# winstonww/ReacherDistilation

Hardware: AMD Instinct MI355X
Metric: Reacher env-steps/sec (rollout+distill step) at 1/2/4/8 MI355X; student MSE (higher is better)
Workload: dtype f32; 1 GPU; c4; description=BASELINE config 4: 262,144 envs per GPU, RCCL student-grad all-reduce, MSE, fp32, envs_per_gpu=262144, envs_total=262144, student=MlpPolicy 2x64 tanh (5060 params, f32), teacher=MlpPolicy 2x64 tanh, loss=mse, act_with=teacher, optimizer=TF1 Adam lr 0.0001, 1 step per env-step, parallelism=dp1, collective=none, f32_mode=split

## Files before the change

### reacherdistilation_amd/csrc/distill_forward.h

```cpp
#pragma once

#ifdef RD_MFMA_SRCC_FENCE
constexpr bool kFenceAll = true;
#else
constexpr bool kFenceAll = false;
#endif
#include "distill_forward_f32.h"

constexpr unsigned kPairFence = 0x8a00u;
template <bool FENCE = false, unsigned FM = FENCE ? 0xffffu : 0u>
__device__ __forceinline__ void mlp_forward_pair(const float* LT, const float* LS, const float* ob, int j, int g,
                                                 f32x4 (&H1)[4], f32x4 (&H2)[4], float& mt0, float& mt1,
                                                 float& ms0, float& ms1) {
    f32x4 at[4], as[4];
#pragma unroll
    for (int fb = 0; fb < 4; ++fb) at[fb] = as[fb] = f32x4{0.f, 0.f, 0.f, 0.f};
#pragma unroll
    for (int s = 0; s < 3; ++s) {
        const int k = 4 * s + g;
        const float x = ob[j * SOS + k];
        const float zt = fminf(fmaxf((x - LT[N_MU + k]) * LT[N_RS + k], -5.0f), 5.0f);
        const float zs = fminf(fmaxf((x - LS[N_MU + k]) * LS[N_RS + k], -5.0f), 5.0f);
        const f32x4 wt = ld4(LT + N_W1 + k * HID + 4 * j);
        const f32x4 ws = ld4(LS + N_W1 + k * HID + 4 * j);
// ... 87 lines not shown
}
__device__ __forceinline__ bf16x8 ldbf8(const float* base, int half) {
    return *reinterpret_cast<const bf16x8*>(reinterpret_cast<const unsigned short*>(base) + half);
}

__device__ __forceinline__ int kperm(int s, int g, int jj) { return 32 * s + 4 * g + (jj & 3) + 16 * (jj >> 2); }

__device__ void load_net_bf16(float* L, const float* g, int nthreads) {
    unsigned short* w1 = reinterpret_cast<unsigned short*>(L + NB_W1);
    unsigned short* w2f = reinterpret_cast<unsigned short*>(L + NB_W2F);
    unsigned short* w2b = reinterpret_cast<unsigned short*>(L + NB_W2B);
    for (int x = threadIdx.x; x < 4 * 4 * 16 * 8; x += nthreads) {
        const int jj = x & 7, i = (x >> 3) & 15, fb = (x >> 7) & 3, gg = x >> 9;
        const int k = 8 * gg + jj;
        w1[x] = bf16_bits(k < OBD ? g[P_W1 + k * HID + 16 * fb + i] : 0.0f);
    }
    for (int x = threadIdx.x; x < 2 * 4 * 4 * 16 * 8; x += nthreads) {
        const int jj = x & 7, i = (x >> 3) & 15, b = (x >> 7) & 3, gg = (x >> 9) & 3, s = x >> 11;
        const int kp = kperm(s, gg, jj);
        w2f[x] = bf16_bits(g[P_W2 + kp * HID + 16 * b + i]);
        w2b[x] = bf16_bits(g[P_W2 + (16 * b + i) * HID + kp]);
    }
    for (int x = threadIdx.x; x < HID; x += nthreads) {
        L[NB_B1 + x] = g[P_B1 + x];
        L[NB_B2 + x] = g[P_B2 + x];
    }
    for (int x = threadIdx.x; x < HID * ACD; x += nthreads) L[NB_W3 + x] = bf16_round(g[P_W3 + x]);
    if (threadIdx.x < ACD) {
        L[NB_B3 + threadIdx.x] = g[P_B3 + threadIdx.x];
        L[NB_LS + threadIdx.x] = g[P_LS + threadIdx.x];
    }
    if (threadIdx.x < 12) {
        const int k = threadIdx.x;
        L[NB_MU + k] = k < OBD ? g[P_TOT + k] : 0.0f;
        L[NB_RS + k] = k < OBD ? 1.0f / g[P_TOT + OBD + k] : 1.0f;
    }
}

typedef unsigned u32x4 __attribute__((ext_vector_type(4)));

__device__ __forceinline__ void split1(float x, unsigned short (&h)[3]) {
    const uint32_t u = __float_as_uint(x);
    const float r = x - __uint_as_float(u & 0xffff0000u);
    const uint32_t ur = __float_as_uint(r);
    const float l = r - __uint_as_float(ur & 0xffff0000u);
    h[0] = (unsigned short)(u >> 16);
    h[1] = (unsigned short)(ur >> 16);
    h[2] = (unsigned short)(__float_as_uint(l) >> 16);
}

__device__ __forceinline__ void split_bits(float x, uint32_t& u0, uint32_t& u1, uint32_t& u2) {
    u0 = __float_as_uint(x);
    const float r = x - __uint_as_float(u0 & 0xffff0000u);
    u1 = __float_as_uint(r);
    u2 = __float_as_uint(r - __uint_as_float(u1 & 0xffff0000u));
}

__device__ __forceinline__ void split8(f32x4 lo, f32x4 hi, bf16x8 (&p)[3]) {
    const float x[8] = {lo[0], lo[1], lo[2], lo[3], hi[0], hi[1], hi[2], hi[3]};
    uint32_t u0[8], u1[8], u2[8];
#pragma unroll
    for (int i = 0; i < 8; ++i) split_bits(x[i], u0[i], u1[i], u2[i]);
    u32x4 q0, q1, q2;
#pragma unroll
    for (int i = 0; i < 4; ++i) {
        q0[i] = __builtin_amdgcn_perm(u0[2 * i + 1], u0[2 * i], 0x07060302u);
        q1[i] = __builtin_amdgcn_perm(u1[2 * i + 1], u1[2 * i], 0x07060302u);
        q2[i] = __builtin_amdgcn_perm(u2[2 * i + 1], u2[2 * i], 0x07060302u);
    }
    p[0] = __builtin_bit_cast(bf16x8, q0);
    p[1] = __builtin_bit_cast(bf16x8, q1);
    p[2] = __builtin_bit_cast(bf16x8, q2);
}

__device__ __forceinline__ uint32_t pair_hi(uint32_t a, uint32_t b) { return __builtin_amdgcn_perm(b, a, 0x07060302u); }

__device__ __forceinline__ f32x4 mfma_split(const bf16x8 (&w)[3], const bf16x8 (&x)[3], f32x4 c) {
    c = mfma_k32(w[2], x[0], c);
    c = mfma_k32(w[1], x[1], c);
    c = mfma_k32(w[0], x[2], c);
    c = mfma_k32(w[1], x[0], c);
    c = mfma_k32(w[0], x[1], c);
    return mfma_k32(w[0], x[0], c);
}

typedef float f32x16 __attribute__((ext_vector_type(16)));
__device__ __forceinline__ f32x16 mfma_32k16(bf16x8 a, bf16x8 b, f32x16 c) {
    return __builtin_amdgcn_mfma_f32_32x32x16_bf16(a, b, c, 0, 0, 0);
}
__device__ __forceinline__ void dw2_split32(const float (&x)[2][8], const float (&y)[2][8], f32x16 (&g)[2][2]) {
    bf16x8 xp[2][3], yp[2][3];
#pragma unroll
    for (int b = 0; b < 2; ++b) {
        split8(f32x4{x[b][0], x[b][1], x[b][2], x[b][3]}, f32x4{x[b][4], x[b][5], x[b][6], x[b][7]}, xp[b]);
        split8(f32x4{y[b][0], y[b][1], y[b][2], y[b][3]}, f32x4{y[b][4], y[b][5], y[b][6], y[b][7]}, yp[b]);
    }
#pragma unroll
    for (int mb = 0; mb < 2; ++mb)
#pragma unroll
        for (int nb = 0; nb < 2; ++nb) {
            f32x16 c = g[mb][nb];
            c = mfma_32k16(xp[mb][2], yp[nb][0], c);
            c = mfma_32k16(xp[mb][1], yp[nb][1], c);
            c = mfma_32k16(xp[mb][0], yp[nb][2], c);
            c = mfma_32k16(xp[mb][1], yp[nb][0], c);
            c = mfma_32k16(xp[mb][0], yp[nb][1], c);
            g[mb][nb] = mfma_32k16(xp[mb][0], yp[nb][0], c);
        }
}

__device__ __forceinline__ void ld_pieces(const float* L, int base, int o, bf16x8 (&w)[3]) {
    const unsigned short* h = reinterpret_cast<const unsigned short*>(L + base);
#pragma unroll
    for (int q = 0; q < 3; ++q) w[q] = *reinterpret_cast<const bf16x8*>(h + q * SP_PIECE + o);
}

__device__ __forceinline__ void layer1_split(const float* L, const float* ob, int j, int g, f32x4 (&acc)[4]) {
    u32x4 b[3];
#pragma unroll
    for (int s = 0; s < 3; ++s) {
        const int k = 4 * s + g;
        const float z = fminf(fmaxf((ob[j * SOS + k] - L[NX_MU + k]) * L[NX_RS + k], -5.0f), 5.0f);
        uint32_t z0, z1, z2;
        split_bits(z, z0, z1, z2);
        b[0][s] = pair_hi(z2, z0);
        b[1][s] = pair_hi(z1, z1);
        b[2][s] = pair_hi(z0, z0);
    }
#pragma unroll
    for (int q = 0; q < 3; ++q) {
        b[q][3] = 0u;
        const bf16x8 bq = __builtin_bit_cast(bf16x8, b[q]);
#pragma unroll
        for (int fb = 0; fb < 4; ++fb)
            acc[fb] = mfma_k32(ldbf8(L + NX_W1S, ((((q ? 1 : 0) * 4 + g) * 4 + fb) * 16 + j) * 8), bq, acc[fb]);
    }
}

__device__ __forceinline__ void mlp_forward_pair_split(const float* LT, const float* LS, const float* ob, int j, int g,
                                                       f32x4 (&H1)[4], f32x4 (&H2)[4], float& mt0, float& mt1,
                                                       float& ms0, float& ms1) {
    f32x4 at[4], as[4];
#pragma unroll
    for (int fb = 0; fb < 4; ++fb) at[fb] = as[fb] = f32x4{0.f, 0.f, 0.f, 0.f};
    layer1_split(LT, ob, j, g, at);
    layer1_split(LS, ob, j, g, as);
    f32x4 T1[4];
#pragma unroll
    for (int fb = 0; fb < 4; ++fb) {
        T1[fb] = tanh4(at[fb]);
        H1[fb] = tanh4(as[fb]);
    }
#pragma unroll
    for (int fb = 0; fb < 4; ++fb) {
        at[fb] = ld4(LT + NX_B2 + 16 * fb + 4 * g);
        as[fb] = ld4(LS + NX_B2 + 16 * fb + 4 * g);
    }
    {
        bf16x8 tp[2][3], sp[2][3];
        __builtin_amdgcn_sched_barrier(0);
        split8(T1[0], T1[1], tp[0]);
        split8(H1[0], H1[1], sp[0]);
        __builtin_amdgcn_sched_barrier(0);
        split8(T1[2], T1[3], tp[1]);
        split8(H1[2], H1[3], sp[1]);
#pragma unroll
// ... 276 lines not shown
```

### reacherdistilation_amd/csrc/distill_layout.h

```cpp
#pragma once

constexpr int OBD = 11, HID = 64, ACD = 2;
constexpr int P_W1 = 0;
constexpr int P_B1 = P_W1 + OBD * HID;
constexpr int P_W2 = P_B1 + HID;
constexpr int P_B2 = P_W2 + HID * HID;
constexpr int P_W3 = P_B2 + HID;
constexpr int P_B3 = P_W3 + HID * ACD;
constexpr int P_LS = P_B3 + ACD;
constexpr int P_TOT = P_LS + ACD;
constexpr int P_PAD = P_TOT + 4;
constexpr int N_MET = 4;

constexpr int WAVES = 8, BLOCK = 64 * WAVES;
constexpr int FWAVES = 4, FBLOCK = 64 * FWAVES;
constexpr int GROUP = 64;
constexpr int TILE = 16;

constexpr int N_W1 = 0;
constexpr int N_W2 = N_W1 + 12 * HID;
constexpr int N_B2 = N_W2 + HID * HID;
constexpr int N_W3 = N_B2 + HID;
constexpr int N_B3 = N_W3 + HID * ACD;
constexpr int N_LS = N_B3 + ACD;
constexpr int N_MU = N_LS + ACD;
constexpr int N_RS = N_MU + 12;
constexpr int NET = (N_RS + 12 + 3) & ~3;
constexpr int N_W2T = NET;
constexpr int NET_S = NET + HID * HID;
static_assert(N_B2 % 4 == 0 && N_W3 % 4 == 0 && NET % 4 == 0, "16-B aligned LDS vectors");

constexpr int PAIRS = WAVES / 2;
constexpr int SOS = 12;
constexpr int SAS = 68;
constexpr int P_SO = 0;
constexpr int P_ACT = P_SO + GROUP * SOS;
constexpr int P_H1T = P_ACT + GROUP * 2;
constexpr int P_DZT = P_H1T + TILE * SAS;
constexpr int P_SA = P_DZT + TILE * SAS;
constexpr int P_SOB = P_SA + TILE * SAS;
constexpr int P_SACT = P_SOB + TILE * SOS;
constexpr int P_FLAGS = P_SACT + TILE * 2;
constexpr int PSCR = P_FLAGS + 4;
constexpr int LDS_FLOATS = NET + NET_S + PAIRS * PSCR;
static_assert(LDS_FLOATS * 4 <= 160 * 1024, "LDS budget");
static_assert(PSCR % 4 == 0 && P_H1T % 4 == 0 && P_DZT % 4 == 0 && P_SA % 4 == 0 && P_SOB % 4 == 0,
              "16-B aligned scratch");
constexpr int RROW = 68;
constexpr int RSHIFT = (P_B2 / HID) * (RROW - HID);
constexpr int RPAD = P_PAD + RSHIFT;
static_assert(P_B1 == P_W1 + OBD * HID && P_W2 == P_B1 + HID && P_B2 % HID == 0, "W1|b1|W2 rows");
static_assert(PAIRS * RPAD <= LDS_FLOATS && RPAD % 4 == 0 && P_PAD % 4 == 0, "final reduction must fit in the LDS");
__device__ __forceinline__ int ridx(int p) { return p < P_B2 ? (p >> 6) * RROW + (p & 63) : p + RSHIFT; }
[[maybe_unused]] constexpr int NSTAMP = 24;
constexpr uint32_t SPIN_LIMIT = 1u << 22;

constexpr int NB_W1 = 0;
constexpr int NB_W2F = NB_W1 + 4 * 4 * 16 * 8 / 2;
constexpr int NB_W2B = NB_W2F + 2 * 4 * 4 * 16 * 8 / 2;
constexpr int NB_B1 = NB_W2B + 2 * 4 * 4 * 16 * 8 / 2;
constexpr int NB_B2 = NB_B1 + HID;
constexpr int NB_W3 = NB_B2 + HID;
constexpr int NB_B3 = NB_W3 + HID * ACD;
constexpr int NB_LS = NB_B3 + ACD;
constexpr int NB_MU = NB_LS + ACD;
constexpr int NB_RS = NB_MU + 12;
constexpr int NETB_S = (NB_RS + 12 + 3) & ~3;
static_assert(NETB_S <= NET_S && NB_B1 % 4 == 0 && NB_W3 % 4 == 0, "bf16 student image");

constexpr int SP_PIECE = 2 * 4 * 4 * 16 * 8;
constexpr int NX_B2 = 0;
constexpr int NX_W3 = NX_B2 + HID;
constexpr int NX_B3 = NX_W3 + HID * ACD;
constexpr int NX_LS = NX_B3 + ACD;
constexpr int NX_MU = NX_LS + ACD;
constexpr int NX_RS = NX_MU + 12;
constexpr int NX_W2F = NX_RS + 12;
constexpr int NX_W1S = NX_W2F + 3 * SP_PIECE / 2;
constexpr int NETX = NX_W1S + 2 * 4 * 4 * 16 * 8 / 2;
constexpr int NX_W2B = NETX;
constexpr int NETX_S = NX_W2B + 3 * SP_PIECE / 2;
static_assert(NX_W3 % 4 == 0 && NX_B2 % 4 == 0 && NX_W2F % 4 == 0 && NX_W1S % 4 == 0 && NETX % 4 == 0 &&
              NETX_S % 4 == 0, "16-B aligned split images");

template <int K> struct Off;
template <> struct Off<0> { static constexpr int W3 = N_W3, MU = N_MU, RS = N_RS; };
template <> struct Off<1> { static constexpr int W3 = NX_W3, MU = NX_MU, RS = NX_RS; };
template <> struct Off<2> { static constexpr int W3 = NB_W3, MU = NB_MU, RS = NB_RS; };

constexpr int img_t(bool SPL) { return SPL ? NETX : NET; }
constexpr int img_s(bool BS, bool SPL) { return BS ? NETB_S : (SPL ? NETX_S : NET_S); }
static_assert((NETX + NETX_S + PAIRS * PSCR) * 4 <= 160 * 1024 && (NETX + NETB_S + PAIRS * PSCR) * 4 <= 160 * 1024,
              "LDS budget (split images)");
```

### reacherdistilation_amd/csrc/distill_rollout.h

```cpp
#pragma once

struct RolloutArgs {
    int64_t n, env_base;
    uint64_t seed;
    float* state;
    const float* tnet;
    const float* snet;
    uint32_t* ctl;
    float* ws;
    int loss, act_student, stagger;
    float inv_n_global;
    int gs;
    int ksteps;
    unsigned long long* dbg;
    const float* obs_in;
    const float* timg;
    const float* simg;
};

__device__ __forceinline__ bool wait_ge(const uint32_t* f, uint32_t target, uint32_t* err) {
    for (uint32_t spins = 0;; ++spins) {
        if (__hip_atomic_load(f, __ATOMIC_ACQUIRE, __HIP_MEMORY_SCOPE_WORKGROUP) >= target) return true;
        if (spins > SPIN_LIMIT) {
            if ((threadIdx.x & 63) == 0) __hip_atomic_store(err, 1u, __ATOMIC_RELAXED, __HIP_MEMORY_SCOPE_AGENT);
            return false;
        }
        __builtin_amdgcn_s_sleep(1);
    }
}

__device__ __forceinline__ void publish(uint32_t* f, uint32_t v) {
    __hip_atomic_store(f, v, __ATOMIC_RELEASE, __HIP_MEMORY_SCOPE_WORKGROUP);
}

__device__ __forceinline__ float env_step_group(const RolloutArgs& a, uint32_t C, int64_t i, bool valid, float act0,
                                                float act1, rd::State& st, float& met_n) {
    const uint32_t iu = (uint32_t)i;
    const float rew = rd::env_step<false>(st, act0, act1);
    const int64_t gid = a.env_base + i;
    const uint32_t u = C + (a.stagger ? (uint32_t)((gid / RDD_STAGGER_GROUP) % rd::kEpisodeSteps) : 0u);
    const bool done_step = (u % rd::kEpisodeSteps) == rd::kEpisodeSteps - 1;
    if (done_step) {
        float dr[6];
        rd::philox_draw(a.seed, (uint64_t)gid, u / rd::kEpisodeSteps + 1, dr);
        rd::env_reset(st, dr);
    }
    if (!valid) return 0.0f;
    rd::store_state(a.state, a.n, iu, st, done_step);
    met_n += 1.0f;
    return rew;
}

constexpr int MD_TEACHER = 0, MD_ROWS = 1, MD_HELPER = 2;
template <bool BS, bool SPL, bool CP, int MD, bool KS = false, bool TC = false>
__global__ __launch_bounds__(BLOCK, 2) void rollout_kernel(RolloutArgs a) {
    constexpr bool TGT = MD == MD_ROWS, HLP = MD == MD_HELPER;
    static_assert(!TC || (BS && MD == MD_TEACHER && !KS), "teacher on the consumer: bf16 student, K = 1");
    constexpr int P_TM = CP ? P_ACT : P_SACT;
    static_assert(!HLP || !BS, "helper pairs: f32 student kernels only");
    constexpr int TN = TGT ? 0 : img_t(SPL), SN = img_s(BS, SPL);
    __shared__ __attribute__((aligned(16))) float lds[TN + SN + PAIRS * PSCR];
    float* LT = lds;
    float* LS = lds + TN;
    const int wave = threadIdx.x >> 6, lane = threadIdx.x & 63;
    const int j = lane & 15, g = lane >> 4;
    const int pair = wave & (PAIRS - 1);
    const bool producer = wave < PAIRS;
    uint32_t* flags = reinterpret_cast<uint32_t*>(lds + TN + SN + pair * PSCR + P_FLAGS);
    uint32_t* err = a.ctl + 8;

    RTSTAMP(16);
    STAMP(0);
    const int gs = a.gs;
    const uint32_t n32 = (uint32_t)a.n;
    const uint32_t ngroups = (n32 + (uint32_t)gs - 1) / (uint32_t)gs;
    static_assert(!KS || (!CP && MD == MD_TEACHER), "K-step launches: teacher mode, producer-side env step");
    if constexpr (KS) {
        if (a.obs_in) {
            if (threadIdx.x == 0) __hip_atomic_store(a.ctl + 8, 1u, __ATOMIC_RELAXED, __HIP_MEMORY_SCOPE_AGENT);
            return;
        }
    }
    if constexpr (HLP) {
        if (ngroups > 2u * gridDim.x) {
            if (threadIdx.x == 0) __hip_atomic_store(a.ctl + 8, 1u, __ATOMIC_RELAXED, __HIP_MEMORY_SCOPE_AGENT);
            return;
        }
    }
    const bool helper = HLP && pair >= 2;
    const uint32_t gstride = gridDim.x * (HLP ? 2 : PAIRS);
    const uint32_t gfirst = helper ? ngroups : blockIdx.x * (HLP ? 2 : PAIRS) + pair;
    rd::State st0{};
    if (producer && !a.obs_in && gfirst < ngroups && lane < gs && gfirst * gs + lane < a.n)
        load_state(a.state, a.n, (uint32_t)(gfirst * gs + lane), st0);
    const uint32_t og = blockIdx.x * 2 + (pair & 1);
    const bool hstep = helper && producer && !a.obs_in && !a.act_student;
    if constexpr (HLP) {
        if (hstep && og < ngroups && lane < gs && og * gs + lane < a.n)
            load_state(a.state, a.n, (uint32_t)(og * gs + lane), st0);
    }
    static_assert(NET % 4 == 0 && NET_S % 4 == 0, "16-B images");
    float* PS = lds + TN + SN + pair * PSCR;
    const bool first_obs = producer && gfirst < ngroups;
    auto group_obs = [&](uint32_t k, uint32_t i, bool lvalid, rd::State& st) {
        float ob[OBD];
        if (a.obs_in) {
#pragma unroll
            for (int q = 0; q < OBD; ++q) ob[q] = lvalid ? a.obs_in[(size_t)i * OBD + q] : 0.0f;
        } else {
            rd::observe<false>(st, ob);
        }
        float* o = PS + P_SO + lane * SOS;
        st4(o, f32x4{ob[0], ob[1], ob[2], ob[3]});
        st4(o + 4, f32x4{ob[4], ob[5], ob[6], ob[7]});
        st4(o + 8, f32x4{ob[8], ob[9], ob[10], 1.0f});
    };
    copy_images<TN / 4, SN / 4, BLOCK>(LT, a.timg, a.simg, [&] {
        if (first_obs) {
            const uint32_t i = gfirst * (uint32_t)gs + (uint32_t)lane;
            group_obs(0, i, lane < gs && i < n32, st0);
        }
    });
    using SO = Off<BS ? IMG_BF16 : (SPL ? IMG_SPLIT : IMG_F32)>;
    constexpr int SW3 = SO::W3, SMU = SO::MU, SRS = SO::RS;
    if (threadIdx.x < PAIRS * 4)
        reinterpret_cast<uint32_t*>(lds + TN + SN + (threadIdx.x >> 2) * PSCR + P_FLAGS)[threadIdx.x & 3] = 0u;

    const uint32_t C = a.ctl[0];
    if (blockIdx.x == 0 && threadIdx.x < 4) a.ctl[4 + threadIdx.x] = a.ctl[threadIdx.x];
    if (blockIdx.x == 0 && threadIdx.x == 4) a.ctl[12] = a.obs_in ? 0u : (KS ? (uint32_t)a.ksteps : 1u);
    __syncthreads();
    STAMP(1);

    if (producer) {
        f32x4 gw3a[4], gw3b[4];
#pragma unroll
        for (int x = 0; x < 4; ++x) gw3a[x] = gw3b[x] = f32x4{0.f, 0.f, 0.f, 0.f};
        float gb3a = 0, gb3b = 0, gls0 = 0, gls1 = 0, met_l = 0, met_m = 0, met_r = 0, met_n = 0;
        const float tl0 = TGT ? 0.0f : a.tnet[P_LS], tl1 = TGT ? 0.0f : a.tnet[P_LS + 1];
        const float sl0 = a.snet[P_LS], sl1 = a.snet[P_LS + 1];
        const float sv0 = __expf(2.0f * sl0), sv1 = __expf(2.0f * sl1);
        const float rtv0 = 1.0f / __expf(2.0f * tl0), rtv1 = 1.0f / __expf(2.0f * tl1);
        uint32_t tiles = 0;
        uint32_t k = 0;
// ... 42 lines not shown
                group_obs(k, i, lvalid, st);
            } else {
                if (!a.obs_in && lvalid) load_state(a.state, a.n, i, st);
                group_obs(k, i, lvalid, st);
            }
            STAMP(11);
            wave_sync();
            if constexpr (TC) publish(flags + 2, k + 1);
            const int ntile = (int)min((uint32_t)(gs / TILE), (n32 - base + TILE - 1) / TILE);
            for (int t = 0; t < ntile; ++t) {
                const bool tvalid = base + TILE * t + j < a.n;
                const float* obt = obs + TILE * t * SOS;
                f32x4 H1[4], H2[4];
                float mt0, mt1, ms0, ms1;
                float rl0 = tl0, rl1 = tl1, rr0 = rtv0, rr1 = rtv1;
                STAMP(10);
                if constexpr (TGT) {
                    const uint32_t row = base + TILE * t + j;
                    const f32x4 tq = tvalid ? ld4(a.tnet + (size_t)row * 4) : f32x4{0.f, 0.f, 0.f, 0.f};
                    if constexpr (BS) mlp_forward_bf16(LS, obt, j, g, H1, H2, ms0, ms1);
                    else if constexpr (SPL) mlp_forward_split_t<true>(LS, obt, j, g, H1, H2, ms0, ms1);
                    else mlp_forward(LS, obt, j, g, H1, H2, ms0, ms1);
                    mt0 = tq[0];
                    mt1 = tq[1];
                    rl0 = tq[2];
                    rl1 = tq[3];
                    rr0 = 1.0f / __expf(2.0f * rl0);
                    rr1 = 1.0f / __expf(2.0f * rl1);
                } else if constexpr (HLP) {
                    if (k == 0) {
                        if constexpr (SPL) mlp_forward_split_t<true>(LS, obt, j, g, H1, H2, ms0, ms1);
                        else mlp_forward<true>(LS, obt, j, g, H1, H2, ms0, ms1);
                        const float* hp = lds + TN + SN + (pair + 2) * PSCR;
                        if (!(ok = wait_ge(reinterpret_cast<const uint32_t*>(hp + P_FLAGS), 1u, err))) break;
                        mt0 = hp[P_ACT + 2 * j];
                        mt1 = hp[P_ACT + 2 * j + 1];
                    } else {
                        if constexpr (SPL) mlp_forward_pair_split(LT, LS, obt, j, g, H1, H2, mt0, mt1, ms0, ms1);
                        else mlp_forward_pair<true>(LT, LS, obt, j, g, H1, H2, mt0, mt1, ms0, ms1);
                    }
                } else if constexpr (BS) {
                    if (TC && (t & 1)) {
                        mlp_forward_bf16(LS, obt, j, g, H1, H2, ms0, ms1);
                        if (!(ok = wait_ge(flags + 3, ++tct, err))) break;
                        mt0 = PS[P_TM + 2 * j];
                        mt1 = PS[P_TM + 2 * j + 1];
                    } else {
                    if constexpr (SPL) mlp_forward_split(LT, obt, j, g, mt0, mt1);
                    else mlp_forward<CP || KS || TC>(LT, obt, j, g, H1, H2, mt0, mt1);
                    mlp_forward_bf16(LS, obt, j, g, H1, H2, ms0, ms1);
                    }
                } else {
                    if constexpr (SPL) mlp_forward_pair_split(LT, LS, obt, j, g, H1, H2, mt0, mt1, ms0, ms1);
                    else mlp_forward_pair<false, kPairFence>(LT, LS, obt, j, g, H1, H2, mt0, mt1, ms0, ms1);
                }
                STAMP(12);
                const float d0 = ms0 - mt0, d1 = ms1 - mt1;
                float dm0, dm1, dl0 = 0.0f, dl1 = 0.0f, lossv;
                if (a.loss == RDD_LOSS_MSE) {
                    dm0 = d0 * a.inv_n_global;
                    dm1 = d1 * a.inv_n_global;
                    lossv = (d0 * d0 + d1 * d1) * (0.5f * a.inv_n_global);
                } else {
                    dm0 = d0 * rr0;
                    dm1 = d1 * rr1;
                    dl0 = sv0 * rr0 - 1.0f;
                    dl1 = sv1 * rr1 - 1.0f;
                    lossv = (rl0 - sl0 + (sv0 + d0 * d0) * (0.5f * rr0) - 0.5f) +
                            (rl1 - sl1 + (sv1 + d1 * d1) * (0.5f * rr1) - 0.5f);
                }
                if (!tvalid) { dm0 = dm1 = dl0 = dl1 = 0.0f; }
                if (g == 0 && tvalid) {
                    met_l += lossv;
                    met_m += d0 * d0 + d1 * d1;
                    gb3a += dm0; gb3b += dm1; gls0 += dl0; gls1 += dl1;
                    if (!CP) {
                        act[(TILE * t + j) * 2] = a.act_student ? ms0 : mt0;
                        act[(TILE * t + j) * 2 + 1] = a.act_student ? ms1 : mt1;
                    }
                }
                f32x4 dZ[4];
#pragma unroll
                for (int fb = 0; fb < 4; ++fb) {
                    const f32x4 wa = ld4(LS + SW3 + (16 * fb + 4 * g) * 2);
                    const f32x4 wb = ld4(LS + SW3 + (16 * fb + 4 * g) * 2 + 4);
                    const float w0[4] = {wa[0], wa[2], wb[0], wb[2]}, w1[4] = {wa[1], wa[3], wb[1], wb[3]};
#pragma unroll
                    for (int r = 0; r < 4; ++r) {
                        const float h = H2[fb][r];
                        gw3a[fb][r] = fmaf(h, dm0, gw3a[fb][r]);
                        gw3b[fb][r] = fmaf(h, dm1, gw3b[fb][r]);
                        dZ[fb][r] = fmaf(w0[r], dm0, w1[r] * dm1) * fmaf(-h, h, 1.0f);
                    }
                }
                STAMP(2);
                if (!(ok = wait_ge(flags + 1, tiles, err))) break;
                STAMP(3);
                float* h1t = PS + P_H1T;
                float* dzt = PS + P_DZT;
#pragma unroll
                for (int fb = 0; fb < 4; ++fb) {
                    st4(h1t + j * SAS + 16 * fb + 4 * g, H1[fb]);
                    st4(dzt + j * SAS + 16 * fb + 4 * g, dZ[fb]);
                }
                if (lane < TILE * SOS / 4) st4(PS + P_SOB + 4 * lane, ld4(obt + 4 * lane));
                if (CP && g == 0) {
                    PS[P_SACT + 2 * j] = a.act_student ? ms0 : mt0;
                    PS[P_SACT + 2 * j + 1] = a.act_student ? ms1 : mt1;
                }
                publish(flags, ++tiles);
            }
            if (!ok) break;
            STAMP(4);
            if constexpr (!CP) {
                if (a.obs_in) {
                    if (lvalid) met_n += 1.0f;
                } else if (HLP && k == 0 && !a.act_student) {
                } else {
                    wave_sync();
                    if (lane < gs) met_r += env_step_group(a, Ck, i, lvalid, act[lane * 2], act[lane * 2 + 1], st, met_n);
                }
            }
            if constexpr (KS) st0 = st;
            STAMP(5);
        }
        if (!KS || !ok || kk + 1 >= K) break;
        }
#pragma unroll
        for (int x = 0; x < 4; ++x)
#pragma unroll
            for (int r = 0; r < 4; ++r)
#pragma unroll
                for (int o = 8; o >= 1; o >>= 1) {
                    gw3a[x][r] += __shfl_xor(gw3a[x][r], o, 16);
                    gw3b[x][r] += __shfl_xor(gw3b[x][r], o, 16);
                }
        gb3a = wave_sum(gb3a); gb3b = wave_sum(gb3b);
        gls0 = wave_sum(gls0); gls1 = wave_sum(gls1);
        met_l = wave_sum(met_l); met_m = wave_sum(met_m);
        met_r = wave_sum(met_r); met_n = wave_sum(met_n);
        STAMP(6);
        __syncthreads();
        STAMP(9);
        float* R = lds + pair * RPAD + RSHIFT;
        if (j == 0) {
#pragma unroll
            for (int fb = 0; fb < 4; ++fb)
#pragma unroll
                for (int r = 0; r < 4; ++r) {
                    const int f = 16 * fb + 4 * g + r;
                    R[P_W3 + 2 * f] = gw3a[fb][r];
                    R[P_W3 + 2 * f + 1] = gw3b[fb][r];
                }
        }
        if (lane == 0) {
            R[P_B3] = gb3a; R[P_B3 + 1] = gb3b; R[P_LS] = gls0; R[P_LS + 1] = gls1;
            R[P_TOT + 1] = met_l; R[P_TOT + 2] = met_m;
            if constexpr (!CP) { R[P_TOT] = met_r; R[P_TOT + 3] = met_n; }
        }
    } else {
        f32x4 gW2[4][4], gW1[4];
        float gb2[4];
        constexpr bool D32 = SPL || BS;
        f32x16 gW2s[2][2];
        float gb2s[2] = {0.f, 0.f};
#pragma unroll
        for (int x = 0; x < 4; ++x) {
#pragma unroll
            for (int y = 0; y < 4; ++y) gW2[x][y] = f32x4{0.f, 0.f, 0.f, 0.f};
            gW1[x] = f32x4{0.f, 0.f, 0.f, 0.f};
            gb2[x] = 0.0f;
        }
#pragma unroll
        for (int x = 0; x < 2; ++x)
#pragma unroll
            for (int y = 0; y < 2; ++y)
#pragma unroll
                for (int r = 0; r < 16; ++r) gW2s[x][y][r] = 0.0f;
        const int c32 = lane & 31, h32 = lane >> 5;
        const float smu = j < 12 ? LS[SMU + j] : 0.0f, srs = j < 12 ? LS[SRS + j] : 0.0f;
        float met_r = 0.0f, met_n = 0.0f;
        uint32_t tiles = 0;
        bool ok = true;
        float act0 = 0.0f, act1 = 0.0f;
        auto bwd_tile = [&](int t) -> bool {
            STAMP(2);
            if (!wait_ge(flags, tiles + 1, err)) return false;
            STAMP(3);
            const float* h1t = PS + P_H1T;
            const float* dzt = PS + P_DZT;
            float xin[4];
#pragma unroll
            for (int e = 0; e < 4; ++e) xin[e] = PS[P_SOB + (BS ? 4 * g + e : 4 * e + g) * SOS + (j < 12 ? j : 0)];
            f32x4 H1[4], dZ[4], acc[4];
            if constexpr (BS) {
                bf16x8 xa8[2], yb8[2];
#pragma unroll
                for (int b = 0; b < 2; ++b) {
                    float xv[8], yv[8];
#pragma unroll
                    for (int e = 0; e < 8; ++e) {
                        xv[e] = h1t[(8 * h32 + e) * SAS + 32 * b + c32];
                        yv[e] = dzt[(8 * h32 + e) * SAS + 32 * b + c32];
                    }
                    gb2s[b] += ((yv[0] + yv[1]) + (yv[2] + yv[3])) + ((yv[4] + yv[5]) + (yv[6] + yv[7]));
                    xa8[b] = pack8(f32x4{xv[0], xv[1], xv[2], xv[3]}, f32x4{xv[4], xv[5], xv[6], xv[7]});
                    yb8[b] = pack8(f32x4{yv[0], yv[1], yv[2], yv[3]}, f32x4{yv[4], yv[5], yv[6], yv[7]});
                }
#pragma unroll
                for (int b = 0; b < 4; ++b) {
                    H1[b] = ld4(h1t + j * SAS + 16 * b + 4 * g);
                    dZ[b] = ld4(dzt + j * SAS + 16 * b + 4 * g);
                }
                if (CP && (lane >> 4) == t) {
                    act0 = PS[P_SACT + 2 * (lane & 15)];
                    act1 = PS[P_SACT + 2 * (lane & 15) + 1];
                }
                publish(flags + 1, ++tiles);
                STAMP(13);
#pragma unroll
                for (int mb = 0; mb < 2; ++mb)
#pragma unroll
                    for (int nb = 0; nb < 2; ++nb) gW2s[mb][nb] = mfma_32k16(xa8[mb], yb8[nb], gW2s[mb][nb]);
#pragma unroll
                for (int mb = 0; mb < 4; ++mb) acc[mb] = f32x4{0.f, 0.f, 0.f, 0.f};
#pragma unroll
                for (int s = 0; s < 2; ++s) {
                    const bf16x8 db = pack8(dZ[2 * s], dZ[2 * s + 1]);
#pragma unroll
                    for (int mb = 0; mb < 4; ++mb)
                        acc[mb] = mfma_k32(ldbf8(LS + NB_W2B, (((s * 4 + g) * 4 + mb) * 16 + j) * 8), db, acc[mb]);
                }
            } else {
                constexpr bool S2 = SPL;
                float x[4][4], y[4][4];
                float x32[2][8], y32[2][8];
                if constexpr (S2) {
#pragma unroll
                    for (int e = 0; e < 8; ++e)
#pragma unroll
                        for (int b = 0; b < 2; ++b) {
                            x32[b][e] = h1t[(8 * h32 + e) * SAS + 32 * b + c32];
                            y32[b][e] = dzt[(8 * h32 + e) * SAS + 32 * b + c32];
                        }
                } else {
#pragma unroll
                for (int s = 0; s < 4; ++s)
#pragma unroll
                    for (int b = 0; b < 4; ++b) {
                        x[s][b] = h1t[(4 * s + g) * SAS + 16 * b + j];
                        y[s][b] = dzt[(4 * s + g) * SAS + 16 * b + j];
                    }
                }
#pragma unroll
                for (int b = 0; b < 4; ++b) {
                    H1[b] = ld4(h1t + j * SAS + 16 * b + 4 * g);
                    dZ[b] = ld4(dzt + j * SAS + 16 * b + 4 * g);
                }
                if (CP && (lane >> 4) == t) {
                    act0 = PS[P_SACT + 2 * (lane & 15)];
                    act1 = PS[P_SACT + 2 * (lane & 15) + 1];
                }
                publish(flags + 1, ++tiles);
                STAMP(13);
                bf16x8 dpre[2][3];
                if constexpr (S2) {
                    if constexpr (!HLP) {
#pragma unroll
                        for (int b = 0; b < 2; ++b)
                            gb2s[b] += ((y32[b][0] + y32[b][1]) + (y32[b][2] + y32[b][3])) +
                                       ((y32[b][4] + y32[b][5]) + (y32[b][6] + y32[b][7]));
                    }
                    split8(dZ[0], dZ[1], dpre[0]);
                    split8(dZ[2], dZ[3], dpre[1]);
                    if constexpr (!HLP) dw2_split32(x32, y32, gW2s);
                } else if constexpr (!HLP) {
#pragma unroll
                for (int s = 0; s < 4; ++s) {
#pragma unroll
                    for (int b = 0; b < 4; ++b) gb2[b] += y[s][b];
#pragma unroll
                    for (int mb = 0; mb < 4; ++mb)
#pragma unroll
                        for (int nb = 0; nb < 4; ++nb) gW2[mb][nb] = mfma(x[s][mb], y[s][nb], gW2[mb][nb]);
                }
                }
#pragma unroll
                for (int mb = 0; mb < 4; ++mb) acc[mb] = f32x4{0.f, 0.f, 0.f, 0.f};
                if constexpr (S2) {
#pragma unroll
                    for (int s = 0; s < 2; ++s) {
#pragma unroll
                        for (int mb = 0; mb < 4; ++mb) {
                            bf16x8 w[3];
                            ld_pieces(LS, NX_W2B, (((s * 4 + g) * 4 + mb) * 16 + j) * 8, w);
                            acc[mb] = mfma_split(w, dpre[s], acc[mb]);
                        }
                    }
                    __builtin_amdgcn_sched_group_barrier(0x002, 40, 0);
#pragma unroll
                    for (int i = 0; i < (HLP ? 48 : 72); ++i) {
                        __builtin_amdgcn_sched_group_barrier(0x008, 1, 0);
                        __builtin_amdgcn_sched_group_barrier(0x002, 3, 0);
                    }
                } else {
                f32x4 wc[4], wn[4];
#pragma unroll
                for (int r = 0; r < 4; ++r) wc[r] = ld4(LS + N_W2T + (4 * g + r) * HID + 4 * j);
#pragma unroll
                for (int fb = 0; fb < 4; ++fb) {
                    if (fb < 3) {
#pragma unroll
                        for (int r = 0; r < 4; ++r) wn[r] = ld4(LS + N_W2T + (16 * (fb + 1) + 4 * g + r) * HID + 4 * j);
                    }
                    fence_begin<true>(acc);
#pragma unroll
                    for (int r = 0; r < 4; ++r)
#pragma unroll
                        for (int mb = 0; mb < 4; ++mb) acc[mb] = mfma(wc[r][mb], dZ[fb][r], acc[mb]);
                    fence_end<true>(acc);
#pragma unroll
                    for (int r = 0; r < 4; ++r) wc[r] = wn[r];
                }
                }
            }
            STAMP(14);
            float* sa = PS + P_SA;
#pragma unroll
            for (int mb = 0; mb < 4; ++mb) {
#pragma unroll
                for (int r = 0; r < 4; ++r) acc[mb][r] *= fmaf(-H1[mb][r], H1[mb][r], 1.0f);
                st4(sa + j * SAS + 16 * mb + 4 * g, acc[mb]);
            }
            wave_sync();
            if constexpr (BS) {
                float zz[4];
#pragma unroll
                for (int jj = 0; jj < 4; ++jj) {
                    zz[jj] = j < 12 ? fminf(fmaxf((xin[jj] - smu) * srs, -5.0f), 5.0f) : 0.0f;
                }
                const s16x4 za = pack4(zz[0], zz[1], zz[2], zz[3]);
#pragma unroll
                for (int nb = 0; nb < 4; ++nb) {
                    const float* c = sa + 16 * nb + j;
                    gW1[nb] = mfma_k16(za, pack4(c[(4 * g) * SAS], c[(4 * g + 1) * SAS], c[(4 * g + 2) * SAS],
                                                 c[(4 * g + 3) * SAS]), gW1[nb]);
                }
            } else {
#pragma unroll
                for (int s = 0; s < 4; ++s) {
                    const float z = j < 12 ? fminf(fmaxf((xin[s] - smu) * srs, -5.0f), 5.0f) : 0.0f;
#pragma unroll
                    for (int nb = 0; nb < 4; ++nb) gW1[nb] = mfma(z, sa[(4 * s + g) * SAS + 16 * nb + j], gW1[nb]);
                }
            }
            wave_sync();
            STAMP(15);
            return true;
        };
        auto end_group = [&](uint32_t base, uint32_t Ck) {
            const uint32_t i = base + (uint32_t)lane;
            const bool lvalid = lane < gs && i < n32;
            if constexpr (CP) {
                STAMP(4);
                if (a.obs_in) {
                    if (lvalid) met_n += 1.0f;
                } else if (lane < gs) {
                    rd::State st{};
                    if (lvalid) load_state(a.state, a.n, i, st);
                    met_r += env_step_group(a, Ck, i, lvalid, act0, act1, st, met_n);
                }
                STAMP(5);
            }
        };
        if constexpr (HLP) {
            if (helper && og < ngroups) {
                const float* OP = lds + TN + SN + (pair & 1) * PSCR;
                STAMP(20);
                ok = wait_ge(reinterpret_cast<const uint32_t*>(OP + P_FLAGS), 1u, err);
                STAMP(21);
                if (ok) {
                    const float* h1t = OP + P_H1T;
                    const float* dzt = OP + P_DZT;
                    if constexpr (SPL) {
                        float x32[2][8], y32[2][8];
#pragma unroll
                        for (int e = 0; e < 8; ++e)
#pragma unroll
                            for (int b = 0; b < 2; ++b) {
                                x32[b][e] = h1t[(8 * h32 + e) * SAS + 32 * b + c32];
                                y32[b][e] = dzt[(8 * h32 + e) * SAS + 32 * b + c32];
                            }
#pragma unroll
                        for (int b = 0; b < 2; ++b)
                            gb2s[b] += ((y32[b][0] + y32[b][1]) + (y32[b][2] + y32[b][3])) +
                                       ((y32[b][4] + y32[b][5]) + (y32[b][6] + y32[b][7]));
                        dw2_split32(x32, y32, gW2s);
                    } else {
                    float x[4][4], y[4][4];
#pragma unroll
                    for (int s = 0; s < 4; ++s)
#pragma unroll
                        for (int b = 0; b < 4; ++b) {
                            x[s][b] = h1t[(4 * s + g) * SAS + 16 * b + j];
                            y[s][b] = dzt[(4 * s + g) * SAS + 16 * b + j];
                        }
#pragma unroll
                        for (int s = 0; s < 4; ++s) {
#pragma unroll
                            for (int b = 0; b < 4; ++b) gb2[b] += y[s][b];
#pragma unroll
                            for (int mb = 0; mb < 4; ++mb) {
                                fence_begin<true>(gW2[mb]);
#pragma unroll
                                for (int nb = 0; nb < 4; ++nb) gW2[mb][nb] = mfma(x[s][mb], y[s][nb], gW2[mb][nb]);
                                fence_end<true>(gW2[mb]);
                            }
                        }
                    }
                }
                STAMP(22);
            }
        }
        uint32_t gi = 0, tcc = 0;
        for (uint32_t kk = 0;; ++kk) {
        for (uint32_t grp = gfirst; ok && grp < ngroups; grp += gstride, ++gi) {
            const uint32_t base = grp * (uint32_t)gs;
            const int ntile = (int)min((uint32_t)(gs / TILE), (n32 - base + TILE - 1) / TILE);
            if constexpr (TC) {
                if (!(ok = wait_ge(flags + 2, gi + 1, err))) break;
            }
            for (int t = 0; ok && t < ntile; ++t) {
                if constexpr (TC) {
                    if (!(t & 1) && t + 1 < ntile) {
                        const float* obt = PS + P_SO + TILE * (t + 1) * SOS;
                        float m0, m1;
                        if constexpr (SPL) {
                            mlp_forward_split(LT, obt, j, g, m0, m1);
                        } else {
                            f32x4 h1[4], h2[4];
                            mlp_forward<true>(LT, obt, j, g, h1, h2, m0, m1);
                        }
                        if (g == 0) {
                            PS[P_TM + 2 * j] = m0;
                            PS[P_TM + 2 * j + 1] = m1;
                        }
                        publish(flags + 3, ++tcc);
                    }
                }
                ok = bwd_tile(t);
            }
            if (!ok) break;
            end_group(base, C + kk);
        }
        if (!KS || !ok || kk + 1 >= (uint32_t)a.ksteps) break;
        }
#pragma unroll
        for (int x = 0; x < 4; ++x) gb2[x] = xsum32(xsum16(gb2[x]));
#pragma unroll
        for (int x = 0; x < 2; ++x) gb2s[x] = xsum32(gb2s[x]);
        if constexpr (CP) { met_r = wave_sum(met_r); met_n = wave_sum(met_n); }
        STAMP(6);
        __syncthreads();
        STAMP(9);
        float* R = lds + pair * RPAD;
        if constexpr (D32) {
#pragma unroll
            for (int mb = 0; mb < 2; ++mb)
#pragma unroll
                for (int nb = 0; nb < 2; ++nb)
#pragma unroll
                    for (int r = 0; r < 16; ++r)
                        R[(12 + 32 * mb + (r & 3) + 8 * (r >> 2) + 4 * h32) * RROW + 32 * nb + c32] = gW2s[mb][nb][r];
        } else {
#pragma unroll
// ... 42 lines not shown
```

Measured before the change: 3.481 billion env-steps/s.

## Defer dZ2 computation to consumer and drop LDS round-trip for layer-1 gradient

For the split-f32 student path, the producer now stores H2 plus the per-row output error dm in scratch instead of computing dZ2. The consumer and helper compute dZ2 from these values. The backward MFMA for W2 is transposed so its accumulator comes out in a register layout that feeds the W1-gradient MFMA directly. This removes the LDS store/reload of the SA tile and its wave syncs. It trades extra per-consumer arithmetic and a reordered scratch layout for less LDS traffic and fewer barriers.

```diff
diff --git a/reacherdistilation_amd/csrc/distill_forward.h b/reacherdistilation_amd/csrc/distill_forward.h
--- a/reacherdistilation_amd/csrc/distill_forward.h
+++ b/reacherdistilation_amd/csrc/distill_forward.h
@@ -193,6 +193,15 @@
     c = mfma_k32(w[1], x[0], c);
     c = mfma_k32(w[0], x[1], c);
     return mfma_k32(w[0], x[0], c);
+}
+
+__device__ __forceinline__ f32x4 mfma_split_t(const bf16x8 (&x)[3], const bf16x8 (&w)[3], f32x4 c) {
+    c = mfma_k32(x[0], w[2], c);
+    c = mfma_k32(x[1], w[1], c);
+    c = mfma_k32(x[2], w[0], c);
+    c = mfma_k32(x[0], w[1], c);
+    c = mfma_k32(x[1], w[0], c);
+    return mfma_k32(x[0], w[0], c);
 }
 
 typedef float f32x16 __attribute__((ext_vector_type(16)));
diff --git a/reacherdistilation_amd/csrc/distill_layout.h b/reacherdistilation_amd/csrc/distill_layout.h
--- a/reacherdistilation_amd/csrc/distill_layout.h
+++ b/reacherdistilation_amd/csrc/distill_layout.h
@@ -37,14 +37,15 @@
 constexpr int P_ACT = P_SO + GROUP * SOS;
 constexpr int P_H1T = P_ACT + GROUP * 2;
 constexpr int P_DZT = P_H1T + TILE * SAS;
-constexpr int P_SA = P_DZT + TILE * SAS;
-constexpr int P_SOB = P_SA + TILE * SAS;
+constexpr int P_SOB = P_DZT + TILE * SAS;
 constexpr int P_SACT = P_SOB + TILE * SOS;
-constexpr int P_FLAGS = P_SACT + TILE * 2;
-constexpr int PSCR = P_FLAGS + 4;
+constexpr int P_DM = P_SACT + TILE * 2;
+constexpr int P_FLAGS = P_DM + TILE * 2;
+constexpr int P_SA = P_FLAGS + 4;
+constexpr int PSCR = P_SA + TILE * SAS;
 constexpr int LDS_FLOATS = NET + NET_S + PAIRS * PSCR;
 static_assert(LDS_FLOATS * 4 <= 160 * 1024, "LDS budget");
-static_assert(PSCR % 4 == 0 && P_H1T % 4 == 0 && P_DZT % 4 == 0 && P_SA % 4 == 0 && P_SOB % 4 == 0,
+static_assert(PSCR % 4 == 0 && P_H1T % 4 == 0 && P_DZT % 4 == 0 && P_SOB % 4 == 0 && P_DM % 4 == 0 && P_SA % 4 == 0,
               "16-B aligned scratch");
 constexpr int RROW = 68;
 constexpr int RSHIFT = (P_B2 / HID) * (RROW - HID);
diff --git a/reacherdistilation_amd/csrc/distill_rollout.h b/reacherdistilation_amd/csrc/distill_rollout.h
--- a/reacherdistilation_amd/csrc/distill_rollout.h
+++ b/reacherdistilation_amd/csrc/distill_rollout.h
@@ -33,6 +33,22 @@
     __hip_atomic_store(f, v, __ATOMIC_RELEASE, __HIP_MEMORY_SCOPE_WORKGROUP);
 }
 
+__device__ __forceinline__ float dz2_value(float w0, float w1, float d0, float d1, float h) {
+#pragma clang fp contract(off)
+    const float u = fmaf(w0, d0, w1 * d1), v = fmaf(-h, h, 1.0f);
+    return u * v;
+}
+
+__device__ __forceinline__ void dz2_from_h2(float (&y)[2][8], const f32x4 (&dme)[4], const float (&w3)[4]) {
+#pragma unroll
+    for (int b = 0; b < 2; ++b)
+#pragma unroll
+        for (int e = 0; e < 8; ++e) {
+            const float h = y[b][e], d0 = dme[e >> 1][2 * (e & 1)], d1 = dme[e >> 1][2 * (e & 1) + 1];
+            y[b][e] = dz2_value(w3[b], w3[2 + b], d0, d1, h);
+        }
+}
+
 __device__ __forceinline__ float env_step_group(const RolloutArgs& a, uint32_t C, int64_t i, bool valid, float act0,
                                                 float act1, rd::State& st, float& met_n) {
     const uint32_t iu = (uint32_t)i;
@@ -55,11 +71,14 @@
 template <bool BS, bool SPL, bool CP, int MD, bool KS = false, bool TC = false>
 __global__ __launch_bounds__(BLOCK, 2) void rollout_kernel(RolloutArgs a) {
     constexpr bool TGT = MD == MD_ROWS, HLP = MD == MD_HELPER;
+    constexpr bool DZC = SPL && !BS;
     static_assert(!TC || (BS && MD == MD_TEACHER && !KS), "teacher on the consumer: bf16 student, K = 1");
     constexpr int P_TM = CP ? P_ACT : P_SACT;
     static_assert(!HLP || !BS, "helper pairs: f32 student kernels only");
     constexpr int TN = TGT ? 0 : img_t(SPL), SN = img_s(BS, SPL);
-    __shared__ __attribute__((aligned(16))) float lds[TN + SN + PAIRS * PSCR];
+    constexpr int LDSN = TN + SN + PAIRS * PSCR > PAIRS * RPAD ? TN + SN + PAIRS * PSCR : PAIRS * RPAD;
+    static_assert(LDSN * 4 <= 160 * 1024, "LDS budget");
+    __shared__ __attribute__((aligned(16))) float lds[LDSN];
     float* LT = lds;
     float* LS = lds + TN;
     const int wave = threadIdx.x >> 6, lane = threadIdx.x & 63;
@@ -268,15 +287,18 @@
                 f32x4 dZ[4];
 #pragma unroll
                 for (int fb = 0; fb < 4; ++fb) {
-                    const f32x4 wa = ld4(LS + SW3 + (16 * fb + 4 * g) * 2);
-                    const f32x4 wb = ld4(LS + SW3 + (16 * fb + 4 * g) * 2 + 4);
+                    f32x4 wa = f32x4{0.f, 0.f, 0.f, 0.f}, wb = wa;
+                    if constexpr (!DZC) {
+                        wa = ld4(LS + SW3 + (16 * fb + 4 * g) * 2);
+                        wb = ld4(LS + SW3 + (16 * fb + 4 * g) * 2 + 4);
+                    }
                     const float w0[4] = {wa[0], wa[2], wb[0], wb[2]}, w1[4] = {wa[1], wa[3], wb[1], wb[3]};
 #pragma unroll
                     for (int r = 0; r < 4; ++r) {
                         const float h = H2[fb][r];
                         gw3a[fb][r] = fmaf(h, dm0, gw3a[fb][r]);
                         gw3b[fb][r] = fmaf(h, dm1, gw3b[fb][r]);
-                        dZ[fb][r] = fmaf(w0[r], dm0, w1[r] * dm1) * fmaf(-h, h, 1.0f);
+                        if constexpr (!DZC) dZ[fb][r] = fmaf(w0[r], dm0, w1[r] * dm1) * fmaf(-h, h, 1.0f);
                     }
                 }
                 STAMP(2);
@@ -287,7 +309,11 @@
 #pragma unroll
                 for (int fb = 0; fb < 4; ++fb) {
                     st4(h1t + j * SAS + 16 * fb + 4 * g, H1[fb]);
-                    st4(dzt + j * SAS + 16 * fb + 4 * g, dZ[fb]);
+                    st4(dzt + j * SAS + 16 * fb + 4 * g, DZC ? H2[fb] : dZ[fb]);
+                }
+                if (DZC && g == 0) {
+                    PS[P_DM + 2 * j] = dm0;
+                    PS[P_DM + 2 * j + 1] = dm1;
                 }
                 if (lane < TILE * SOS / 4) st4(PS + P_SOB + 4 * lane, ld4(obt + 4 * lane));
                 if (CP && g == 0) {
@@ -364,6 +390,14 @@
 #pragma unroll
                 for (int r = 0; r < 16; ++r) gW2s[x][y][r] = 0.0f;
         const int c32 = lane & 31, h32 = lane >> 5;
+        float w3y[4] = {0.f, 0.f, 0.f, 0.f};
+        if constexpr (DZC) {
+#pragma unroll
+            for (int b = 0; b < 2; ++b) {
+                w3y[b] = LS[SW3 + (32 * b + c32) * 2];
+                w3y[2 + b] = LS[SW3 + (32 * b + c32) * 2 + 1];
+            }
+        }
         const float smu = j < 12 ? LS[SMU + j] : 0.0f, srs = j < 12 ? LS[SRS + j] : 0.0f;
         float met_r = 0.0f, met_n = 0.0f;
         uint32_t tiles = 0;
@@ -378,7 +412,10 @@
             float xin[4];
 #pragma unroll
             for (int e = 0; e < 4; ++e) xin[e] = PS[P_SOB + (BS ? 4 * g + e : 4 * e + g) * SOS + (j < 12 ? j : 0)];
-            f32x4 H1[4], dZ[4], acc[4];
+            constexpr bool TR = SPL || BS;
+            const int pj = !TR ? j : BS ? j : 4 * (j & 3) + (j >> 2);
+            f32x4 dZ[4], acc[4];
+            float h1e[4][4];
             if constexpr (BS) {
                 bf16x8 xa8[2], yb8[2];
 #pragma unroll
@@ -395,8 +432,9 @@
                 }
 #pragma unroll
                 for (int b = 0; b < 4; ++b) {
-                    H1[b] = ld4(h1t + j * SAS + 16 * b + 4 * g);
-                    dZ[b] = ld4(dzt + j * SAS + 16 * b + 4 * g);
+                    dZ[b] = ld4(dzt + pj * SAS + 16 * b + 4 * g);
+#pragma unroll
+                    for (int r = 0; r < 4; ++r) h1e[b][r] = h1t[(4 * g + r) * SAS + 16 * b + j];
                 }
                 if (CP && (lane >> 4) == t) {
                     act0 = PS[P_SACT + 2 * (lane & 15)];
@@ -415,19 +453,21 @@
                     const bf16x8 db = pack8(dZ[2 * s], dZ[2 * s + 1]);
 #pragma unroll
                     for (int mb = 0; mb < 4; ++mb)
-                        acc[mb] = mfma_k32(ldbf8(LS + NB_W2B, (((s * 4 + g) * 4 + mb) * 16 + j) * 8), db, acc[mb]);
+                        acc[mb] = mfma_k32(db, ldbf8(LS + NB_W2B, (((s * 4 + g) * 4 + mb) * 16 + j) * 8), acc[mb]);
                 }
             } else {
                 constexpr bool S2 = SPL;
                 float x[4][4], y[4][4];
                 float x32[2][8], y32[2][8];
+                bf16x8 dpre[2][3];
                 if constexpr (S2) {
 #pragma unroll
                     for (int e = 0; e < 8; ++e)
 #pragma unroll
                         for (int b = 0; b < 2; ++b) {
                             x32[b][e] = h1t[(8 * h32 + e) * SAS + 32 * b + c32];
-                            y32[b][e] = dzt[(8 * h32 + e) * SAS + 32 * b + c32];
+                            if constexpr (!HLP)
+                                y32[b][e] = dzt[(8 * h32 + e) * SAS + 32 * b + c32];
                         }
                 } else {
 #pragma unroll
@@ -440,8 +480,22 @@
                 }
 #pragma unroll
                 for (int b = 0; b < 4; ++b) {
-                    H1[b] = ld4(h1t + j * SAS + 16 * b + 4 * g);
-                    dZ[b] = ld4(dzt + j * SAS + 16 * b + 4 * g);
+                    dZ[b] = ld4(dzt + pj * SAS + 16 * b + 4 * g);
+#pragma unroll
+                    for (int r = 0; r < 4; ++r) {
+                        if constexpr (S2) h1e[b][r] = h1t[(4 * r + g) * SAS + 16 * b + j];
+                        else h1e[b][r] = h1t[j * SAS + 16 * b + 4 * g + r];
+                    }
+                }
+                f32x4 dme[4];
+                float dmp0 = 0.0f, dmp1 = 0.0f;
+                if constexpr (DZC) {
+                    if constexpr (!HLP) {
+#pragma unroll
+                        for (int q = 0; q < 4; ++q) dme[q] = ld4(PS + P_DM + 16 * h32 + 4 * q);
+                    }
+                    dmp0 = PS[P_DM + 2 * pj];
+                    dmp1 = PS[P_DM + 2 * pj + 1];
                 }
                 if (CP && (lane >> 4) == t) {
                     act0 = PS[P_SACT + 2 * (lane & 15)];
@@ -449,7 +503,19 @@
                 }
                 publish(flags + 1, ++tiles);
                 STAMP(13);
-                bf16x8 dpre[2][3];
+                if constexpr (DZC) {
+                    if constexpr (!HLP) dz2_from_h2(y32, dme, w3y);
+#pragma unroll
+                    for (int fb = 0; fb < 4; ++fb) {
+                        const f32x4 wa = ld4(LS + SW3 + (16 * fb + 4 * g) * 2);
+                        const f32x4 wb = ld4(LS + SW3 + (16 * fb + 4 * g) * 2 + 4);
+                        const float w0[4] = {wa[0], wa[2], wb[0], wb[2]}, w1[4] = {wa[1], wa[3], wb[1], wb[3]};
+#pragma unroll
+                        for (int r = 0; r < 4; ++r) {
+                            dZ[fb][r] = dz2_value(w0[r], w1[r], dmp0, dmp1, dZ[fb][r]);
+                        }
+                    }
+                }
                 if constexpr (S2) {
                     if constexpr (!HLP) {
 #pragma unroll
@@ -480,7 +546,7 @@
                         for (int mb = 0; mb < 4; ++mb) {
                             bf16x8 w[3];
                             ld_pieces(LS, NX_W2B, (((s * 4 + g) * 4 + mb) * 16 + j) * 8, w);
-                            acc[mb] = mfma_split(w, dpre[s], acc[mb]);
+                            acc[mb] = mfma_split_t(dpre[s], w, acc[mb]);
                         }
                     }
                     __builtin_amdgcn_sched_group_barrier(0x002, 40, 0);
@@ -511,14 +577,16 @@
                 }
             }
             STAMP(14);
+#pragma unroll
+            for (int mb = 0; mb < 4; ++mb)
+#pragma unroll
+                for (int r = 0; r < 4; ++r) acc[mb][r] *= fmaf(-h1e[mb][r], h1e[mb][r], 1.0f);
             float* sa = PS + P_SA;
-#pragma unroll
-            for (int mb = 0; mb < 4; ++mb) {
-#pragma unroll
-                for (int r = 0; r < 4; ++r) acc[mb][r] *= fmaf(-H1[mb][r], H1[mb][r], 1.0f);
-                st4(sa + j * SAS + 16 * mb + 4 * g, acc[mb]);
-            }
-            wave_sync();
+            if constexpr (!TR) {
+#pragma unroll
+                for (int mb = 0; mb < 4; ++mb) st4(sa + j * SAS + 16 * mb + 4 * g, acc[mb]);
+                wave_sync();
+            }
             if constexpr (BS) {
                 float zz[4];
 #pragma unroll
@@ -527,20 +595,18 @@
                 }
                 const s16x4 za = pack4(zz[0], zz[1], zz[2], zz[3]);
 #pragma unroll
-                for (int nb = 0; nb < 4; ++nb) {
-                    const float* c = sa + 16 * nb + j;
-                    gW1[nb] = mfma_k16(za, pack4(c[(4 * g) * SAS], c[(4 * g + 1) * SAS], c[(4 * g + 2) * SAS],
-                                                 c[(4 * g + 3) * SAS]), gW1[nb]);
-                }
+                for (int nb = 0; nb < 4; ++nb)
+                    gW1[nb] = mfma_k16(za, pack4(acc[nb][0], acc[nb][1], acc[nb][2], acc[nb][3]), gW1[nb]);
             } else {
 #pragma unroll
                 for (int s = 0; s < 4; ++s) {
                     const float z = j < 12 ? fminf(fmaxf((xin[s] - smu) * srs, -5.0f), 5.0f) : 0.0f;
 #pragma unroll
-                    for (int nb = 0; nb < 4; ++nb) gW1[nb] = mfma(z, sa[(4 * s + g) * SAS + 16 * nb + j], gW1[nb]);
-                }
-            }
-            wave_sync();
+                    for (int nb = 0; nb < 4; ++nb)
+                        gW1[nb] = mfma(z, TR ? acc[nb][s] : sa[(4 * s + g) * SAS + 16 * nb + j], gW1[nb]);
+                }
+            }
+            if constexpr (!TR) wave_sync();
             STAMP(15);
             return true;
         };
@@ -577,6 +643,12 @@
                                 x32[b][e] = h1t[(8 * h32 + e) * SAS + 32 * b + c32];
                                 y32[b][e] = dzt[(8 * h32 + e) * SAS + 32 * b + c32];
                             }
+                        if constexpr (DZC) {
+                            f32x4 dme[4];
+#pragma unroll
+                            for (int q = 0; q < 4; ++q) dme[q] = ld4(OP + P_DM + 16 * h32 + 4 * q);
+                            dz2_from_h2(y32, dme, w3y);
+                        }
 #pragma unroll
                         for (int b = 0; b < 2; ++b)
                             gb2s[b] += ((y32[b][0] + y32[b][1]) + (y32[b][2] + y32[b][3])) +
```

Result: no change. 3.512 billion env-steps/s, median of 6 (+0.9%).
